# jcyk/gtos

Hardware: AMD Instinct MI355X
Metric: graphs/sec training step (100-node AMR, batch 64) (higher is better)
Workload: dtype bf16

## Files before the change

### gtos_amd/csrc/gemm.hip

```cpp
#include "common.h"
#include <stdlib.h>

__attribute__((visibility("hidden"))) const void* gtos_zero_block() {
    static void* z = nullptr;
    if (!z) {
        if (hipMalloc(&z, 256) != hipSuccess) return nullptr;
        if (hipMemset(z, 0, 256) != hipSuccess) return nullptr;
    }
    return z;
}

namespace {

constexpr int BM = 128, BN = 128;
constexpr int ROWB = 128;

template <typename T> struct GemmCfg;
template <> struct GemmCfg<bf16_t> { static constexpr int BK = 64, VEC = 8; };
template <> struct GemmCfg<float>  { static constexpr int BK = 32, VEC = 4; };

template <int NTH> struct TCfg {
    static constexpr int NT = NTH, WAVES_N = NTH / 128, WTN = BN / WAVES_N, NTW = WTN / 16;
    static constexpr int ITERS = 1024 / NTH;
};

inline const void* zero_block() { return gtos_zero_block(); }

struct GemmArgs {
    const void* A; const void* B; void* C; const float* bias;
    int M, N, K; int64_t lda, ldb, ldc;
    int vecA, vecB, vecC;
    int relu, accumulate, splitk;
    float p_drop; uint64_t seed;
    const void* zeros;
    float* ws;
};

__device__ __forceinline__ int swz(int row) { return ((row >> 1) & 7) ^ ((row >> 4) & 3); }
__device__ __forceinline__ int lds_off(int r, int c) { return r * ROWB + ((c ^ swz(r)) << 4); }

template <typename T, bool KC, bool FAST, int NTH>
__device__ __forceinline__ void load_tile(const T* __restrict__ base, const U128* __restrict__ zeros, int64_t ld, int rows_total,
                                          int row0, int k0, int kend, U128 (&regs)[TCfg<NTH>::ITERS]) {
    constexpr int VEC = GemmCfg<T>::VEC, NT = NTH, ITERS = TCfg<NTH>::ITERS;
#pragma unroll
    for (int it = 0; it < ITERS; ++it) {
        int r, k;
        if (KC) { const int v = it * NT + threadIdx.x; r = row0 + (v >> 3); k = k0 + (v & 7) * VEC; }
        else {
            const int rc = threadIdx.x % (BM / VEC), kq = threadIdx.x / (BM / VEC);
            r = row0 + rc * VEC; k = k0 + kq * ITERS + it;
        }
        if constexpr (FAST) {
            const bool ok = KC ? (r < rows_total && k + VEC <= kend) : (k < kend && r + VEC <= rows_total);
            const int64_t off = KC ? ((int64_t)r * ld + k) : ((int64_t)k * ld + r);
            const U128* p = ok ? reinterpret_cast<const U128*>(base + off) : zeros;
            regs[it] = *p;
        } else {
            U128 val = {0u, 0u, 0u, 0u};
#pragma unroll
            for (int i = 0; i < VEC; ++i) {
                const bool ok = KC ? (r < rows_total && k + i < kend) : (k < kend && r + i < rows_total);
                uint32_t bits = 0u;
                if (ok) {
                    const T x = KC ? base[(int64_t)r * ld + k + i] : base[(int64_t)k * ld + r + i];
                    if constexpr (sizeof(T) == 2) bits = (uint32_t)x; else bits = __float_as_uint(x);
                }
                if constexpr (sizeof(T) == 2) val[i >> 1] |= bits << (16 * (i & 1)); else val[i] = bits;
            }
            regs[it] = val;
        }
    }
}

template <typename T, int NTH>
__device__ __forceinline__ void glds_tile(const T* __restrict__ base, const U128* __restrict__ zeros, int64_t ld, int rows_total,
                                          int row0, int k0, int kend, char* lds_tile) {
    constexpr int VEC = GemmCfg<T>::VEC, NT = NTH, ITERS = TCfg<NTH>::ITERS;
    const int wave = __builtin_amdgcn_readfirstlane(threadIdx.x >> 6), lane = threadIdx.x & 63;
#pragma unroll
    for (int it = 0; it < ITERS; ++it) {
        const int blk = it * (NT / 64) + wave;
        const int rl = blk * 8 + (lane >> 3);
        const int c = (lane & 7) ^ swz(rl);
        const int r = row0 + rl, k = k0 + c * VEC;
        const bool ok = r < rows_total && k + VEC <= kend;
        const void* src = ok ? static_cast<const void*>(base + (int64_t)r * ld + k) : static_cast<const void*>(zeros);
        __builtin_amdgcn_global_load_lds((const __attribute__((address_space(1))) void*)src,
                                         (__attribute__((address_space(3))) void*)(lds_tile + blk * 1024), 16, 0, 0);
    }
}

typedef __attribute__((ext_vector_type(4))) short s16x4_t;

template <typename T, int NTH>
__device__ __forceinline__ void glds_tile_km(const T* __restrict__ base, const U128* __restrict__ zeros, int64_t ld, int rows_total,
                                             int row0, int k0, int kend, char* lds_tile) {
    static_assert(sizeof(T) == 2, "transpose-read path is bf16 only");
    constexpr int NT = NTH, ITERS = TCfg<NTH>::ITERS;
    const int wave = __builtin_amdgcn_readfirstlane(threadIdx.x >> 6), lane = threadIdx.x & 63;
#pragma unroll
    for (int it = 0; it < ITERS; ++it) {
        const int blk = it * (NT / 64) + wave;
        const int kr = lane >> 4, pp = lane & 15;
        const int lp = ((((pp >> 1) ^ kr) & 7) << 1) | (pp & 1);
        const int k = k0 + blk * 4 + kr, r = row0 + lp * 8;
        const bool ok = k < kend && r + 8 <= rows_total;
        const void* src = ok ? static_cast<const void*>(base + (int64_t)k * ld + r) : static_cast<const void*>(zeros);
        __builtin_amdgcn_global_load_lds((const __attribute__((address_space(1))) void*)src,
                                         (__attribute__((address_space(3))) void*)(lds_tile + blk * 1024), 16, 0, 0);
    }
}

__device__ __forceinline__ bf16x8_t tr_fragment(const char* tile, int c0, int ks, int fr, int fq) {
    const int kq = fr >> 2;
    const int col = (((c0 >> 4) ^ kq) << 5) + (fr & 3) * 8;
    const char* p0 = tile + (ks * 32 + fq * 8 + kq) * 256 + col;
    const s16x4_t lo = __builtin_amdgcn_ds_read_tr16_b64_v4i16((__attribute__((address_space(3))) s16x4_t*)(p0));
    const s16x4_t hi = __builtin_amdgcn_ds_read_tr16_b64_v4i16((__attribute__((address_space(3))) s16x4_t*)(p0 + 4 * 256));
    const s16x8_t v = {lo[0], lo[1], lo[2], lo[3], hi[0], hi[1], hi[2], hi[3]};
    return __builtin_bit_cast(bf16x8_t, v);
}

template <typename T, bool KC, int NTH>
__device__ __forceinline__ void store_tile(char* __restrict__ lds, const U128 (&regs)[TCfg<NTH>::ITERS]) {
    constexpr int VEC = GemmCfg<T>::VEC, NT = NTH, ITERS = TCfg<NTH>::ITERS;
    if (KC) {
#pragma unroll
        for (int it = 0; it < ITERS; ++it) {
            const int v = it * NT + threadIdx.x;
            *reinterpret_cast<U128*>(lds + lds_off(v >> 3, v & 7)) = regs[it];
        }
    } else {
        const int rc = threadIdx.x % (BM / VEC), kq = threadIdx.x / (BM / VEC);
        const int kk = kq * ITERS;
        if constexpr (sizeof(T) == 2) {
#pragma unroll
            for (int i = 0; i < 8; ++i) {
                const int w = i >> 1;
                char* dst = lds + lds_off(rc * 8 + i, kk >> 3) + (kk & 7) * 2;
                uint32_t lo, hi = 0u;
                if (i & 1) lo = (regs[0][w] >> 16) | (regs[1][w] & 0xffff0000u);
                else       lo = (regs[0][w] & 0xffffu) | (regs[1][w] << 16);
                if constexpr (ITERS == 4) {
                    if (i & 1) hi = (regs[2][w] >> 16) | (regs[3][w] & 0xffff0000u);
                    else       hi = (regs[2][w] & 0xffffu) | (regs[3][w] << 16);
                    *reinterpret_cast<uint2*>(dst) = make_uint2(lo, hi);
                } else {
                    *reinterpret_cast<uint32_t*>(dst) = lo;
                }
            }
        } else {
#pragma unroll
            for (int i = 0; i < 4; ++i) {
                char* dst = lds + lds_off(rc * 4 + i, kk >> 2) + (kk & 3) * 4;
                if constexpr (ITERS == 4) {
                    const U128 o = {regs[0][i], regs[1][i], regs[2][i], regs[3][i]};
                    *reinterpret_cast<U128*>(dst) = o;
                } else {
                    *reinterpret_cast<uint2*>(dst) = make_uint2(regs[0][i], regs[1][i]);
                }
            }
        }
    }
}

template <typename T, typename TO, bool TA, bool TB, bool FAST, int NTH, int STAGES>
__global__ __launch_bounds__(NTH, 4) void gemm_kernel(GemmArgs a) {
    if (a.p_drop > 0.f) a.seed = live_seed(a.seed);
    constexpr int BK = GemmCfg<T>::BK;
    constexpr int NT = NTH, WAVES_N = TCfg<NTH>::WAVES_N, WTN = TCfg<NTH>::WTN, NTW = TCfg<NTH>::NTW, ITERS = TCfg<NTH>::ITERS;
    constexpr int STAGE = (BM + BN) * ROWB;
    constexpr bool BF = sizeof(T) == 2;
    constexpr bool GA = FAST && (!TA || BF), GB = FAST && (TB || BF);
    constexpr bool TRA = GA && TA, TRB = GB && !TB;
    __shared__ __attribute__((aligned(16))) char lds[STAGES * STAGE];

    const int lane = threadIdx.x & 63, wave = threadIdx.x >> 6;
    const int wm = (wave / WAVES_N) * 64, wn = (wave % WAVES_N) * WTN;
    const int nN = (a.N + BN - 1) / BN;
    int m0, n0, bz;
    const int xcd = blockIdx.x & 7, sq = blockIdx.x >> 3;
    if (a.splitk > 1) {
        const int nM = (a.M + BM - 1) / BM, tiles = nM * nN;
        bz = (sq / tiles) * 8 + xcd;
        const int t = sq % tiles;
        m0 = (t / nN) * BM; n0 = (t % nN) * BN;
        if (bz >= a.splitk) return;
    } else {
        bz = 0;
        m0 = ((sq / nN) * 8 + xcd) * BM; n0 = (sq % nN) * BN;
        if (m0 >= a.M) return;
    }
    const int ktiles = (a.K + BK - 1) / BK;
    const int tps = (ktiles + a.splitk - 1) / a.splitk;
    const int kbeg = bz * tps * BK;
    const int kend = min(a.K, kbeg + tps * BK);
    if (kbeg >= kend && a.splitk > 1) return;

    const T* A = static_cast<const T*>(a.A);
    const T* B = static_cast<const T*>(a.B);
    const U128* Z = static_cast<const U128*>(a.zeros);

    f32x4_t acc[4][NTW];
#pragma unroll
    for (int i = 0; i < 4; ++i)
#pragma unroll
        for (int j = 0; j < NTW; ++j) acc[i][j] = f32x4_t{0.f, 0.f, 0.f, 0.f};

    const int fr = lane & 15, fq = lane >> 4;
    auto dma_a = [&](int k0x, char* dst) {
        if constexpr (TRA) glds_tile_km<T, NTH>(A, Z, a.lda, a.M, m0, k0x, kend, dst);
        else glds_tile<T, NTH>(A, Z, a.lda, a.M, m0, k0x, kend, dst);
    };
    auto dma_b = [&](int k0x, char* dst) {
        if constexpr (TRB) glds_tile_km<T, NTH>(B, Z, a.ldb, a.N, n0, k0x, kend, dst);
        else glds_tile<T, NTH>(B, Z, a.ldb, a.N, n0, k0x, kend, dst);
    };
    auto mma_stage = [&](const char* As, const char* Bs) {
        if constexpr (sizeof(T) == 2) {
#pragma unroll
            for (int ks = 0; ks < 2; ++ks) {
                bf16x8_t fa[4], fb[NTW];
#pragma unroll
                for (int t = 0; t < 4; ++t) {
                    if constexpr (TRA) fa[t] = tr_fragment(As, wm + t * 16, ks, fr, fq);
                    else fa[t] = *reinterpret_cast<const bf16x8_t*>(As + lds_off(wm + t * 16 + fr, ks * 4 + fq));
                }
#pragma unroll
                for (int t = 0; t < NTW; ++t) {
                    if constexpr (TRB) fb[t] = tr_fragment(Bs, wn + t * 16, ks, fr, fq);
                    else fb[t] = *reinterpret_cast<const bf16x8_t*>(Bs + lds_off(wn + t * 16 + fr, ks * 4 + fq));
                }
#pragma unroll
                for (int mt = 0; mt < 4; ++mt)
#pragma unroll
                    for (int nt = 0; nt < NTW; ++nt)
                        acc[mt][nt] = __builtin_amdgcn_mfma_f32_16x16x32_bf16(fb[nt], fa[mt], acc[mt][nt], 0, 0, 0);
            }
        } else {
#pragma unroll
            for (int ks = 0; ks < 8; ++ks) {
                float fa[4], fb[NTW];
#pragma unroll
                for (int t = 0; t < 4; ++t) fa[t] = *reinterpret_cast<const float*>(As + lds_off(wm + t * 16 + fr, ks) + fq * 4);
#pragma unroll
                for (int t = 0; t < NTW; ++t) fb[t] = *reinterpret_cast<const float*>(Bs + lds_off(wn + t * 16 + fr, ks) + fq * 4);
#pragma unroll
                for (int mt = 0; mt < 4; ++mt)
#pragma unroll
                    for (int nt = 0; nt < NTW; ++nt)
                        acc[mt][nt] = __builtin_amdgcn_mfma_f32_16x16x4f32(fb[nt], fa[mt], acc[mt][nt], 0, 0, 0);
            }
        }
    };

    if constexpr (STAGES == 1) {
        static_assert(!(STAGES == 1) || (GA && GB), "single-stage variant needs both operands by DMA");
        if constexpr (!TRA && !TRB) {
            const char* Ab = reinterpret_cast<const char*>(A + (int64_t)m0 * a.lda);
            const char* Bb = reinterpret_cast<const char*>(B + (int64_t)n0 * a.ldb);
            const int amax = a.M - 1 - m0, bmax = a.N - 1 - n0;
            const uint32_t lda2 = (uint32_t)a.lda * (uint32_t)sizeof(T), ldb2 = (uint32_t)a.ldb * (uint32_t)sizeof(T);
            const int wv = __builtin_amdgcn_readfirstlane(threadIdx.x >> 6);
            uint32_t offA[ITERS], offB[ITERS];
            int cc[ITERS];
#pragma unroll
            for (int it = 0; it < ITERS; ++it) {
                const int rl = (it * (NT / 64) + wv) * 8 + (lane >> 3);
                cc[it] = (lane & 7) ^ swz(rl);
                offA[it] = (uint32_t)min(rl, amax) * lda2 + (uint32_t)(cc[it] << 4);
                offB[it] = (uint32_t)min(rl, bmax) * ldb2 + (uint32_t)(cc[it] << 4);
            }
            constexpr int VEC = GemmCfg<T>::VEC;
            for (int k0 = kbeg; k0 < kend; k0 += BK) {
                const char* ak = Ab + (int64_t)k0 * (int)sizeof(T);
                const char* bk = Bb + (int64_t)k0 * (int)sizeof(T);
                if (k0 + BK <= kend) {
#pragma unroll
                    for (int it = 0; it < ITERS; ++it) {
                        const int blk = it * (NT / 64) + wv;
                        __builtin_amdgcn_global_load_lds((const __attribute__((address_space(1))) void*)(ak + offA[it]),
                                                         (__attribute__((address_space(3))) void*)(lds + blk * 1024), 16, 0, 0);
                        __builtin_amdgcn_global_load_lds((const __attribute__((address_space(1))) void*)(bk + offB[it]),
                                                         (__attribute__((address_space(3))) void*)(lds + BM * ROWB + blk * 1024), 16, 0, 0);
                    }
                } else {
#pragma unroll
                    for (int it = 0; it < ITERS; ++it) {
                        const int blk = it * (NT / 64) + wv;
                        const bool ok = k0 + cc[it] * VEC + VEC <= kend;
                        const void* sa = ok ? static_cast<const void*>(ak + offA[it]) : static_cast<const void*>(Z);
                        const void* sb = ok ? static_cast<const void*>(bk + offB[it]) : static_cast<const void*>(Z);
                        __builtin_amdgcn_global_load_lds((const __attribute__((address_space(1))) void*)sa,
                                                         (__attribute__((address_space(3))) void*)(lds + blk * 1024), 16, 0, 0);
                        __builtin_amdgcn_global_load_lds((const __attribute__((address_space(1))) void*)sb,
                                                         (__attribute__((address_space(3))) void*)(lds + BM * ROWB + blk * 1024), 16, 0, 0);
                    }
                }
                __syncthreads();
                mma_stage(lds, lds + BM * ROWB);
                __syncthreads();
            }
        } else {
        for (int k0 = kbeg; k0 < kend; k0 += BK) {
            dma_a(k0, lds);
            dma_b(k0, lds + BM * ROWB);
            __syncthreads();
            mma_stage(lds, lds + BM * ROWB);
            __syncthreads();
        }
        }
    } else {
    U128 ra0[ITERS], rb0[ITERS], ra1[ITERS], rb1[ITERS];
    if constexpr (GA) dma_a(kbeg, lds);
    else { load_tile<T, !TA, FAST, NTH>(A, Z, a.lda, a.M, m0, kbeg, kend, ra0); store_tile<T, !TA, NTH>(lds, ra0);
           load_tile<T, !TA, FAST, NTH>(A, Z, a.lda, a.M, m0, kbeg + BK, kend, ra0); }
    if constexpr (GB) dma_b(kbeg, lds + BM * ROWB);
    else { load_tile<T, TB, FAST, NTH>(B, Z, a.ldb, a.N, n0, kbeg, kend, rb0); store_tile<T, TB, NTH>(lds + BM * ROWB, rb0);
           load_tile<T, TB, FAST, NTH>(B, Z, a.ldb, a.N, n0, kbeg + BK, kend, rb0); }
    __syncthreads();

    int cur = 0;
    for (int k0 = kbeg; k0 < kend; k0 += 2 * BK) {
        {
            const char* As = lds + cur * STAGE;
            char* An = lds + (cur ^ 1) * STAGE;
            if constexpr (GA) dma_a(k0 + BK, An);
            else load_tile<T, !TA, FAST, NTH>(A, Z, a.lda, a.M, m0, k0 + 2 * BK, kend, ra1);
            if constexpr (GB) dma_b(k0 + BK, An + BM * ROWB);
            else load_tile<T, TB, FAST, NTH>(B, Z, a.ldb, a.N, n0, k0 + 2 * BK, kend, rb1);
            __builtin_amdgcn_sched_barrier(0);
            mma_stage(As, As + BM * ROWB);
            __builtin_amdgcn_sched_barrier(0);
            if constexpr (!GA) store_tile<T, !TA, NTH>(An, ra0);
            if constexpr (!GB) store_tile<T, TB, NTH>(An + BM * ROWB, rb0);
            __syncthreads();
            cur ^= 1;
        }
        if (k0 + BK >= kend) break;
        {
            const char* As = lds + cur * STAGE;
            char* An = lds + (cur ^ 1) * STAGE;
            if constexpr (GA) dma_a(k0 + 2 * BK, An);
            else load_tile<T, !TA, FAST, NTH>(A, Z, a.lda, a.M, m0, k0 + 3 * BK, kend, ra0);
            if constexpr (GB) dma_b(k0 + 2 * BK, An + BM * ROWB);
            else load_tile<T, TB, FAST, NTH>(B, Z, a.ldb, a.N, n0, k0 + 3 * BK, kend, rb0);
            __builtin_amdgcn_sched_barrier(0);
            mma_stage(As, As + BM * ROWB);
            __builtin_amdgcn_sched_barrier(0);
            if constexpr (!GA) store_tile<T, !TA, NTH>(An, ra1);
            if constexpr (!GB) store_tile<T, TB, NTH>(An + BM * ROWB, rb1);
            __syncthreads();
            cur ^= 1;
        }
    }

    }

    TO* C = static_cast<TO*>(a.C);
    const float keep_scale = a.p_drop > 0.f ? 1.f / (1.f - a.p_drop) : 1.f;

    if constexpr (sizeof(TO) == 2) {
        if (a.vecC && a.splitk == 1) {
            constexpr int CP = WTN * 2 + 16;
            constexpr int LPR = WTN / 8, RPP = 64 / LPR;
            char* cs = lds + wave * 32 * CP;
            if (!a.bias && !a.relu && !(a.p_drop > 0.f) && !a.accumulate && m0 + BM <= a.M && n0 + BN <= a.N) {
                const int rrow = lane / LPR, rcol = (lane % LPR) * 8;
                char* wr = cs + fr * CP + fq * 8;
                const char* rd = cs + rrow * CP + rcol * 2;
                bf16_t* cp0 = reinterpret_cast<bf16_t*>(C) + (int64_t)(m0 + wm + rrow) * a.ldc + n0 + wn + rcol;
#pragma unroll
                for (int half = 0; half < 2; ++half) {
#pragma unroll
                    for (int mh = 0; mh < 2; ++mh)
#pragma unroll
                        for (int nt = 0; nt < NTW; ++nt) {
                            const f32x4_t v = acc[half * 2 + mh][nt];
                            *reinterpret_cast<uint2*>(wr + mh * 16 * CP + nt * 32) = make_uint2(pack_bf(v[0], v[1]), pack_bf(v[2], v[3]));
                        }
                    __builtin_amdgcn_fence(__ATOMIC_RELEASE, "wavefront");
                    __builtin_amdgcn_s_waitcnt(0xc07f);
#pragma unroll
                    for (int pass = 0; pass < 32 / RPP; ++pass) {
                        const uint4 val = *reinterpret_cast<const uint4*>(rd + pass * RPP * CP);
                        *reinterpret_cast<uint4*>(cp0 + (int64_t)(half * 32 + pass * RPP) * a.ldc) = val;
                    }
                    __builtin_amdgcn_s_waitcnt(0xc07f);
                }
                return;
            }
#pragma unroll
            for (int half = 0; half < 2; ++half) {
                if (half) __syncthreads();
#pragma unroll
                for (int mh = 0; mh < 2; ++mh)
#pragma unroll
                    for (int nt = 0; nt < NTW; ++nt) {
                        const int mt = half * 2 + mh;
                        const int m = m0 + wm + mt * 16 + fr, n = n0 + wn + nt * 16 + fq * 4;
                        float v[4] = {acc[mt][nt][0], acc[mt][nt][1], acc[mt][nt][2], acc[mt][nt][3]};
#pragma unroll
                        for (int i = 0; i < 4; ++i) {
                            if (a.bias && n + i < a.N) v[i] += a.bias[n + i];
                            if (a.relu) v[i] = fmaxf(v[i], 0.f);
                            if (a.p_drop > 0.f)
                                v[i] = drop_keep(a.seed, (uint64_t)m * (uint64_t)a.N + (uint64_t)(n + i), a.p_drop) ? v[i] * keep_scale : 0.f;
                        }
                        *reinterpret_cast<uint2*>(cs + (mh * 16 + fr) * CP + (nt * 16 + fq * 4) * 2) =
                            make_uint2(pack_bf(v[0], v[1]), pack_bf(v[2], v[3]));
                    }
                __syncthreads();
#pragma unroll
                for (int pass = 0; pass < 32 / RPP; ++pass) {
                    const int row = pass * RPP + lane / LPR, col = (lane % LPR) * 8;
                    const int m = m0 + wm + half * 32 + row, n = n0 + wn + col;
                    if (m >= a.M || n >= a.N) continue;
                    uint4 val = *reinterpret_cast<const uint4*>(cs + row * CP + col * 2);
                    bf16_t* cp = reinterpret_cast<bf16_t*>(C) + (int64_t)m * a.ldc + n;
                    if (n + 8 <= a.N) {
                        if (a.accumulate) {
                            const uint4 old = *reinterpret_cast<const uint4*>(cp);
                            val = make_uint4(pack_bf(lo_bf(val.x) + lo_bf(old.x), hi_bf(val.x) + hi_bf(old.x)),
                                             pack_bf(lo_bf(val.y) + lo_bf(old.y), hi_bf(val.y) + hi_bf(old.y)),
                                             pack_bf(lo_bf(val.z) + lo_bf(old.z), hi_bf(val.z) + hi_bf(old.z)),
                                             pack_bf(lo_bf(val.w) + lo_bf(old.w), hi_bf(val.w) + hi_bf(old.w)));
                        }
                        *reinterpret_cast<uint4*>(cp) = val;
                    } else {
                        const bf16_t* e = reinterpret_cast<const bf16_t*>(cs + row * CP + col * 2);
                        for (int i = 0; i < 8 && n + i < a.N; ++i) {
                            float o = bf2f(e[i]);
                            if (a.accumulate) o += bf2f(cp[i]);
                            cp[i] = f2bf(o);
                        }
                    }
                }
            }
            return;
        }
    }

#pragma unroll
    for (int mt = 0; mt < 4; ++mt) {
        const int m = m0 + wm + mt * 16 + fr;
        if (m >= a.M) continue;
#pragma unroll
        for (int nt = 0; nt < NTW; ++nt) {
            const int n = n0 + wn + nt * 16 + fq * 4;
            if (n >= a.N) continue;
            float v[4] = {acc[mt][nt][0], acc[mt][nt][1], acc[mt][nt][2], acc[mt][nt][3]};
            TO* cp = C + (int64_t)m * a.ldc + n;
            if (a.splitk > 1) {
                if constexpr (sizeof(TO) == 4) {
                    if (a.ws) {
                        *reinterpret_cast<float4*>(a.ws + ((int64_t)bz * a.M + m) * a.N + n) = make_float4(v[0], v[1], v[2], v[3]);
                    } else {
#pragma unroll
                        for (int i = 0; i < 4; ++i) if (n + i < a.N) atomicAdd(reinterpret_cast<float*>(cp) + i, v[i]);
                    }
                }
                continue;
            }
#pragma unroll
            for (int i = 0; i < 4; ++i) {
                if (a.bias && n + i < a.N) v[i] += a.bias[n + i];
                if (a.relu) v[i] = fmaxf(v[i], 0.f);
                if (a.p_drop > 0.f)
                    v[i] = drop_keep(a.seed, (uint64_t)m * (uint64_t)a.N + (uint64_t)(n + i), a.p_drop) ? v[i] * keep_scale : 0.f;
            }
            if (sizeof(TO) == 4 && a.vecC && n + 3 < a.N) {
                float4 o = make_float4(v[0], v[1], v[2], v[3]);
                if (a.accumulate) { const float4 c = *reinterpret_cast<const float4*>(cp); o.x += c.x; o.y += c.y; o.z += c.z; o.w += c.w; }
                *reinterpret_cast<float4*>(cp) = o;
            } else {
#pragma unroll
                for (int i = 0; i < 4; ++i) if (n + i < a.N) {
                    float o = v[i];
                    if (a.accumulate) o += to_f<TO>(cp[i]);
                    cp[i] = from_f<TO>(o);
                }
            }
        }
    }
}

__global__ void splitk_reduce_kernel(const float* __restrict__ ws, int splits, int M, int N, float* __restrict__ C, int64_t ldc) {
    const int64_t n4 = N / 4, total = (int64_t)M * n4, plane = (int64_t)M * N;
    for (int64_t t = (int64_t)blockIdx.x * blockDim.x + threadIdx.x; t < total; t += (int64_t)gridDim.x * blockDim.x) {
        const int m = (int)(t / n4), n = (int)(t % n4) * 4;
        const float* p = ws + (int64_t)m * N + n;
        float4 acc = *reinterpret_cast<const float4*>(p);
        for (int s = 1; s < splits; ++s) {
            const float4 v = *reinterpret_cast<const float4*>(p + s * plane);
            acc.x += v.x; acc.y += v.y; acc.z += v.z; acc.w += v.w;
        }
        float* cp = C + (int64_t)m * ldc + n;
        cp[0] += acc.x; cp[1] += acc.y; cp[2] += acc.z; cp[3] += acc.w;
    }
}


constexpr int BM2 = 256, BN2 = 256, STAGE2 = (BM2 + BN2) * ROWB;
const bool g_use256 = !(getenv("GTOS_GEMM256") && getenv("GTOS_GEMM256")[0] == '0');

__global__ __launch_bounds__(512, 2) void gemm256_nt_kernel(GemmArgs a) {
    if (a.p_drop > 0.f) a.seed = live_seed(a.seed);
    extern __shared__ __attribute__((aligned(16))) char lds2[];
    const int lane = threadIdx.x & 63, wave = __builtin_amdgcn_readfirstlane(threadIdx.x >> 6);
    const int fr = lane & 15, fq = lane >> 4;
    const int wm = (wave >> 2) * 128, wn = (wave & 3) * 64;
// ... 386 lines not shown
        GTOS_DMA1(ok0 ? pb : Z, (stage) + A3 + wave * 1024);                                                                  \
        GTOS_DMA1(ok1 ? pb + b16 : Z, (stage) + A3 + (8 + wave) * 1024);                                                      \
        kcur += 32; pa += 2 * a16; pb += 2 * b16;                                                                             \
    }
#define GTOS_TRF(tile, c0)                                                                                                    \
    ([&]() -> bf16x8_t {                                                                                                      \
        const char* p0 = (tile) + fbase + ((((c0) >> 4) ^ kq) << 5);                                                          \
        const s16x4_t lo = __builtin_amdgcn_ds_read_tr16_b64_v4i16((__attribute__((address_space(3))) s16x4_t*)(p0));         \
        const s16x4_t hi = __builtin_amdgcn_ds_read_tr16_b64_v4i16((__attribute__((address_space(3))) s16x4_t*)(p0 + 4 * 512)); \
        const s16x8_t v = {lo[0], lo[1], lo[2], lo[3], hi[0], hi[1], hi[2], hi[3]};                                           \
        return __builtin_bit_cast(bf16x8_t, v);                                                                               \
    }())
#define GTOS_STEP(slot_s, slot_d, s_)                                                                                         \
    {                                                                                                                         \
        GTOS_DMA4(slot_d);                                                                                                  \
        _Pragma("unroll") for (int t = 0; t < 4; ++t) fb[t] = GTOS_TRF((slot_s) + A3, wn + t * 16);                           \
        _Pragma("unroll") for (int t = 0; t < 8; ++t) fa[t] = GTOS_TRF((slot_s), wm + t * 16);                                \
        __builtin_amdgcn_s_waitcnt(0x0078);                 \
        __builtin_amdgcn_s_barrier();                                                                                         \
        __builtin_amdgcn_sched_barrier(0);                                                                                    \
        _Pragma("unroll") for (int mt = 0; mt < 8; ++mt)                                                                      \
            _Pragma("unroll") for (int nt = 0; nt < 4; ++nt)                                                                  \
                acc[mt][nt] = __builtin_amdgcn_mfma_f32_16x16x32_bf16(fb[nt], fa[mt], acc[mt][nt], 0, 0, 0);                  \
        __builtin_amdgcn_sched_barrier(0);                                                                                    \
        __builtin_amdgcn_s_barrier();                                                                                         \
    }

    GTOS_DMA4(st0);
    GTOS_DMA4(st1);
    GTOS_DMA4(st2);
    GTOS_VMCNT(8);
    __builtin_amdgcn_s_barrier();
    if (wave >= 4) __builtin_amdgcn_s_barrier();
    int s = 0;
    for (; s + 4 <= nk; s += 4) {
        GTOS_STEP(st0, st3, s);
        GTOS_STEP(st1, st0, s + 1);
        GTOS_STEP(st2, st1, s + 2);
        GTOS_STEP(st3, st2, s + 3);
    }
    if (s < nk) {
        GTOS_STEP(st0, st3, s);
        if (s + 1 < nk) {
            GTOS_STEP(st1, st0, s + 1);
            if (s + 2 < nk) GTOS_STEP(st2, st1, s + 2);
        }
    }
    if (wave < 4) __builtin_amdgcn_s_barrier();
#undef GTOS_STEP
#undef GTOS_TRF
#undef GTOS_DMA4
#undef GTOS_DMA1

#pragma unroll
    for (int mt = 0; mt < 8; ++mt) {
        const int m = m0 + wm + mt * 16 + fr;
        if (m >= a.M) continue;
#pragma unroll
        for (int nt = 0; nt < 4; ++nt) {
            const int n = n0 + wn + nt * 16 + fq * 4;
            if (n >= Nv) continue;
            float4* dst = reinterpret_cast<float4*>(wst + (int64_t)(m - m0) * wld + (n - n0));
            if constexpr (MODE == 2) {
                const float4 o = *dst;
                *dst = make_float4(o.x + acc[mt][nt][0], o.y + acc[mt][nt][1], o.z + acc[mt][nt][2], o.w + acc[mt][nt][3]);
            } else {
                *dst = make_float4(acc[mt][nt][0], acc[mt][nt][1], acc[mt][nt][2], acc[mt][nt][3]);
            }
        }
    }
}

struct ColJob { const bf16_t* A; float* out; int lda, M, K, blk_end, gx; };
struct ColBatch { int njobs, nblocks, rpb; ColJob job[TN_MAX_JOBS]; };
__global__ __launch_bounds__(256) void colsum_batch_kernel(ColBatch g) {
    __shared__ float red[4][64][8];
    int t_ = blockIdx.x, j = 0;
    if (t_ >= g.nblocks) return;
    while (j + 1 < g.njobs && t_ >= g.job[j].blk_end) ++j;
    const ColJob& jb = g.job[j];
    const int tl = t_ - (j ? g.job[j - 1].blk_end : 0);
    const int bx = tl % jb.gx, by = tl / jb.gx;
    const int lane = threadIdx.x & 63, w = threadIdx.x >> 6;
    const int c = (bx * 64 + lane) * 8;
    const int r0 = by * g.rpb, r1 = min(jb.K, r0 + g.rpb);
    float acc[8] = {0, 0, 0, 0, 0, 0, 0, 0};
    if (c < jb.M) {
        for (int r = r0 + w; r < r1; r += 4) {
            float v[8];
            Vec8<bf16_t>::load(jb.A + (int64_t)r * jb.lda + c, v);
#pragma unroll
            for (int e = 0; e < 8; ++e) acc[e] += v[e];
        }
    }
#pragma unroll
    for (int e = 0; e < 8; ++e) red[w][lane][e] = acc[e];
    __syncthreads();
    if (w == 0 && c < jb.M) {
#pragma unroll
        for (int e = 0; e < 8; ++e) atomicAdd(jb.out + c + e, red[0][lane][e] + red[1][lane][e] + red[2][lane][e] + red[3][lane][e]);
    }
}

struct GruDwOut { float* dwih; int64_t ld_ih; float* dwhh; int64_t ld_hh; int hs, in_dim; };
__global__ void gru_dw_reduce_kernel(const float* __restrict__ ws, int splits, TnGroup g, GruDwOut o) {
    const int t_ = blockIdx.x >> 6, q = (blockIdx.x & 63) * 256 + threadIdx.x;
    const int e = g.tmn[t_], src = (e >> 8) & 255;
    const int r = q >> 6, c = (q & 63) * 4;
    const int i = (e & 255) * BM2 + r, j = ((e >> 16) & 255) * BN2 + c;
    if (i >= 4 * o.hs) return;
    const int gate = i / o.hs, ch = i - gate * o.hs;
    float* dst;
    if (src == 0) {
        if (gate == 3 || j >= o.in_dim) return;
        dst = o.dwih + (int64_t)(gate * o.hs + ch) * o.ld_ih + j;
    } else {
        if (gate == 2 || j >= o.hs) return;
        dst = o.dwhh + (int64_t)((gate == 3 ? 2 : gate) * o.hs + ch) * o.ld_hh + j;
    }
    const float* p = ws + (int64_t)t_ * (BM2 * BN2) + r * BN2 + c;
    const int64_t plane = (int64_t)g.tiles * (BM2 * BN2);
    float4 acc = *reinterpret_cast<const float4*>(p);
    for (int s = 1; s < splits; ++s) {
        const float4 v = *reinterpret_cast<const float4*>(p + s * plane);
        acc.x += v.x; acc.y += v.y; acc.z += v.z; acc.w += v.w;
    }
    dst[0] += acc.x; dst[1] += acc.y; dst[2] += acc.z; dst[3] += acc.w;
}

int launch256p_tn(const GemmArgs& a, hipStream_t s) {
    const long long tiles = ((long long)(a.M + BM2 - 1) / BM2) * ((a.N + BN2 - 1) / BN2);
    const long long nblk = tiles * 8 * ((a.splitk + 7) / 8);
    if (nblk > 0x7fffffffLL) return -6;
    hipLaunchKernelGGL((gemm256p_tn_kernel<0, TnGroup>), dim3((unsigned)nblk), dim3(512), 0, s, a, TnGroup{});
    GTOS_CHECK_LAUNCH();
    return 0;
}

int launch256(const GemmArgs& a, hipStream_t s) {
    static bool configured = false;
    if (!configured) {
        if (hipFuncSetAttribute(reinterpret_cast<const void*>(gemm256_nt_kernel), hipFuncAttributeMaxDynamicSharedMemorySize,
                                2 * STAGE2) != hipSuccess) return -7;
        configured = true;
    }
    const long long nMt = (a.M + BM2 - 1) / BM2, nNt = (a.N + BN2 - 1) / BN2;
    const long long nblk = ((nMt + 7) / 8) * 8 * nNt;
    if (nblk > 0x7fffffffLL) return -6;
    hipLaunchKernelGGL(gemm256_nt_kernel, dim3((unsigned)nblk), dim3(512), 2 * STAGE2, s, a);
    GTOS_CHECK_LAUNCH();
    return 0;
}

template <typename T, typename TO>
int launch(const GemmArgs& a, int transA, int transB, hipStream_t s) {
    const long long nMt = (a.M + BM - 1) / BM, nNt = (a.N + BN - 1) / BN;
    const long long nblk = a.splitk > 1 ? nMt * nNt * 8 * ((a.splitk + 7) / 8) : ((nMt + 7) / 8) * 8 * nNt;
    if (nblk > 0x7fffffffLL) return -6;
    dim3 grid((unsigned)nblk);
    const bool fast = a.vecA && a.vecB;
    constexpr bool BF = sizeof(T) == 2;
    if (!transA && transB) {
        if (fast) hipLaunchKernelGGL((gemm_kernel<T, TO, false, true, true, 256, 1>), grid, dim3(256), 0, s, a);
        else      hipLaunchKernelGGL((gemm_kernel<T, TO, false, true, false, 512, 2>), grid, dim3(512), 0, s, a);
    } else if (!transA && !transB) {
        if (fast && BF) hipLaunchKernelGGL((gemm_kernel<T, TO, false, false, true, 256, BF ? 1 : 2>), grid, dim3(256), 0, s, a);
        else if (fast)  hipLaunchKernelGGL((gemm_kernel<T, TO, false, false, true, 512, 2>), grid, dim3(512), 0, s, a);
        else            hipLaunchKernelGGL((gemm_kernel<T, TO, false, false, false, 512, 2>), grid, dim3(512), 0, s, a);
    } else if (transA && !transB) {
        if (fast && BF) hipLaunchKernelGGL((gemm_kernel<T, TO, true, false, true, 256, BF ? 1 : 2>), grid, dim3(256), 0, s, a);
        else if (fast)  hipLaunchKernelGGL((gemm_kernel<T, TO, true, false, true, 512, 2>), grid, dim3(512), 0, s, a);
        else            hipLaunchKernelGGL((gemm_kernel<T, TO, true, false, false, 512, 2>), grid, dim3(512), 0, s, a);
    } else return -2;
    GTOS_CHECK_LAUNCH();
    return 0;
}

}

extern "C" int gtos_gemm(int in_dtype, int out_dtype, int transA, int transB, int M, int N, int K,
                         const void* A, int64_t lda, const void* B, int64_t ldb, void* C, int64_t ldc,
                         const float* bias, int relu, float p_drop, uint64_t seed, int accumulate,
                         int splitk, void* workspace, int64_t workspace_bytes, void* stream) {
    if (M <= 0 || N <= 0) return 0;
    if (K <= 0) return -3;
    const int es = in_dtype == GTOS_BF16 ? 2 : 4, vec = 16 / es;
    const int eo = out_dtype == GTOS_BF16 ? 2 : 4;
    GemmArgs a;
    a.A = A; a.B = B; a.C = C; a.bias = bias; a.M = M; a.N = N; a.K = K; a.lda = lda; a.ldb = ldb; a.ldc = ldc;
    a.vecA = ((uintptr_t)A % 16 == 0) && (lda % vec == 0) && ((transA ? M : K) % vec == 0);
    a.vecB = ((uintptr_t)B % 16 == 0) && (ldb % vec == 0) && ((transB ? K : N) % vec == 0);
    a.vecC = ((uintptr_t)C % 16 == 0) && (ldc % (16 / eo) == 0);
    a.relu = relu; a.accumulate = accumulate; a.p_drop = p_drop; a.seed = seed;
    a.zeros = zero_block();
    if (!a.zeros) return -5;
    if (splitk < 1) splitk = 1;
    const int BKc = in_dtype == GTOS_BF16 ? GemmCfg<bf16_t>::BK : GemmCfg<float>::BK;
    const int ktiles = (K + BKc - 1) / BKc;
    if (splitk > ktiles) splitk = ktiles;
    if (splitk > 1) { const int tps = (ktiles + splitk - 1) / splitk; splitk = (ktiles + tps - 1) / tps; }
    a.splitk = splitk;
    if (splitk > 1 && (out_dtype != GTOS_F32 || bias || relu || p_drop > 0.f || !accumulate)) return -4;
    hipStream_t s = static_cast<hipStream_t>(stream);
    a.ws = nullptr;
    if (splitk > 1 && workspace && N % 4 == 0 && (uintptr_t)workspace % 16 == 0 && (uintptr_t)C % 4 == 0 &&
        (int64_t)splitk * M * N * 4 <= workspace_bytes) {
        a.ws = static_cast<float*>(workspace);
        const int kps = ((ktiles + splitk - 1) / splitk) * BKc;
        const bool tn256 = g_use_pipe_tn && in_dtype == GTOS_BF16 && transA && !transB && a.vecA && a.vecB && M >= 256 && N >= 256 &&
                           M % 8 == 0 && N % 8 == 0 && kps >= 256;
        int rc = tn256 ? launch256p_tn(a, s)
                       : (in_dtype == GTOS_BF16 ? launch<bf16_t, float>(a, transA, transB, s) : launch<float, float>(a, transA, transB, s));
        if (rc) return rc;
        const int64_t total = (int64_t)M * (N / 4);
        const int nb = (int)((total + 255) / 256 < 2048 ? (total + 255) / 256 : 2048);
        hipLaunchKernelGGL(splitk_reduce_kernel, dim3(nb), dim3(256), 0, s, a.ws, splitk, M, N, static_cast<float*>(C), ldc);
        GTOS_CHECK_LAUNCH();
        return 0;
    }
    if (in_dtype == GTOS_BF16 && out_dtype == GTOS_BF16) {
        const long long t256 = ((long long)(M + BM2 - 1) / BM2) * ((N + BN2 - 1) / BN2);
        if (g_use_pipe && !transA && transB && a.vecA && a.vecB && a.vecC && splitk == 1 && N >= 256 && K % 32 == 0 &&
            lda < (1 << 22) && ldb < (1 << 22) &&
            (t256 >= 512 && K >= g_min_kpipe))
            return launch256p(a, s);
        if (g_use256 && !transA && transB && a.vecA && a.vecB && a.vecC && splitk == 1 && t256 >= 1024 && N >= 256 && K >= g_min_k256)
            return launch256(a, s);
        return launch<bf16_t, bf16_t>(a, transA, transB, s);
    }
    if (in_dtype == GTOS_BF16 && out_dtype == GTOS_F32)  return launch<bf16_t, float>(a, transA, transB, s);
    if (in_dtype == GTOS_F32 && out_dtype == GTOS_F32)   return launch<float, float>(a, transA, transB, s);
    return -1;
}


extern "C" int gtos_gru_weight_grads(int rows, int hs, int in_dim, int in_valid, const void* d4, const void* x, int64_t ldx, const void* hprev, int64_t ldh,
                                     float* dwih, int64_t ld_dwih, float* dwhh, int64_t ld_dwhh, void* workspace, int64_t workspace_bytes,
                                     void* stream) {
    if (rows <= 0) return 0;
    if (hs <= 0 || hs % 64 || in_dim < 8 || in_dim % 8 || ldx < in_dim || ldx % 8 || ldh < hs || ldh % 8 || in_valid < 1 || in_valid > in_dim ||
        in_valid % 4) return -22;
    if (!d4 || !x || !hprev || !dwih || !dwhh || !workspace) return -23;
    if ((uintptr_t)d4 % 16 || (uintptr_t)x % 16 || (uintptr_t)hprev % 16 || (uintptr_t)dwih % 4 || (uintptr_t)dwhh % 4 || (uintptr_t)workspace % 16 ||
        ld_dwih < in_valid || ld_dwhh < hs) return -25;
    GemmArgs a{};
    a.A = d4; a.lda = 4 * (int64_t)hs; a.M = 4 * hs; a.B = x; a.ldb = ldx; a.N = in_dim; a.K = rows; a.vecA = a.vecB = 1;
    a.accumulate = 1; a.zeros = zero_block();
    if (!a.zeros) return -5;
    TnGroup g{};
    g.B1 = static_cast<const bf16_t*>(hprev); g.ldb1 = ldh; g.N1 = hs;
    int nt = 0;
    for (int mb = 0; mb * BM2 < 4 * hs; ++mb) {
        const int lo = mb * BM2, hi = (lo + BM2 < 4 * hs ? lo + BM2 : 4 * hs) - 1;
        const int g_lo = lo / hs, g_hi = hi / hs;
        const bool needs_x = g_lo <= 2, needs_h = !(g_lo == 2 && g_hi == 2);
        for (int src = 0; src < 2; ++src) {
            if (!(src ? needs_h : needs_x)) continue;
            const int ncols = src ? hs : in_dim;
            for (int nb = 0; nb * BN2 < ncols; ++nb) {
                if (nt >= 64) return -28;
                g.tmn[nt++] = mb | (src << 8) | (nb << 16);
            }
        }
    }
    g.tiles = nt;
    const int ktiles = (rows + 63) / 64;
    const long long tile_bytes = (long long)BM2 * BN2 * 4;
    long long sk = 8LL * (32 / nt > 0 ? 32 / nt : 1);
    if (sk > ktiles / 4) sk = ktiles / 4;
    if (sk * nt * tile_bytes > workspace_bytes) sk = workspace_bytes / (nt * tile_bytes);
    if (sk < 1) { if (nt * tile_bytes > workspace_bytes) return -4; sk = 1; }
    const int tps = (int)((ktiles + sk - 1) / sk);
    a.splitk = (ktiles + tps - 1) / tps;
    a.ws = static_cast<float*>(workspace);
    hipStream_t s = static_cast<hipStream_t>(stream);
    const long long nblk = (long long)nt * 8 * ((a.splitk + 7) / 8);
    hipLaunchKernelGGL((gemm256p_tn_kernel<1, TnGroup>), dim3((unsigned)nblk), dim3(512), 0, s, a, g);
    GTOS_CHECK_LAUNCH();
    GruDwOut o{dwih, ld_dwih, dwhh, ld_dwhh, hs, in_valid};
    hipLaunchKernelGGL(gru_dw_reduce_kernel, dim3((unsigned)(nt * 64)), dim3(256), 0, s, a.ws, a.splitk, g, o);
    GTOS_CHECK_LAUNCH();
    return 0;
}

extern "C" int gtos_gemm_tn_batch(int n, const void* const* A, const int64_t* lda, const int* M, const void* const* B, const int64_t* ldb,
                                  const int* N, const int* K, float* const* C, const int64_t* ldc, float* const* bias, void* stream) {
    if (n <= 0) return 0;
    if (!A || !lda || !M || !B || !ldb || !N || !K || !C || !ldc) return -23;
    hipStream_t s = static_cast<hipStream_t>(stream);
    const void* zeros = zero_block();
    if (!zeros) return -5;
    for (int j = 0; j < n; ++j) {
        if (M[j] < 8 || M[j] % 8 || N[j] < 8 || N[j] % 8 || K[j] < 1 || lda[j] < M[j] || lda[j] % 8 || ldb[j] < N[j] || ldb[j] % 8 || ldc[j] < N[j] ||
            ldc[j] % 4 || lda[j] >= (1LL << 31) || ldb[j] >= (1LL << 31) || ldc[j] >= (1LL << 31)) return -22;
        if (!A[j] || !B[j] || !C[j] || (uintptr_t)A[j] % 16 || (uintptr_t)B[j] % 16 || (uintptr_t)C[j] % 16) return -25;
        if (bias && bias[j] && (uintptr_t)bias[j] % 4) return -25;
    }
    for (int j0 = 0, nj = 0; j0 < n; j0 += nj) {
        nj = 0;
        while (nj < TN_MAX_JOBS && j0 + nj < n) {
            const int q = j0 + nj;
            const uintptr_t lo = (uintptr_t)C[q], hi = lo + (uintptr_t)(((int64_t)(M[q] - 1) * ldc[q] + N[q]) * 4);
            bool meets = false;
            for (int p = j0; p < q && !meets; ++p) {
                const uintptr_t plo = (uintptr_t)C[p], phi = plo + (uintptr_t)(((int64_t)(M[p] - 1) * ldc[p] + N[p]) * 4);
                meets = lo < phi && plo < hi;
            }
            if (meets) break;
            ++nj;
        }
        TnBatch tb{};
        ColBatch cb{};
        int tiles = 0, blocks = 0, ncol = 0;
        cb.rpb = 512;
        for (int j = 0; j < nj; ++j) {
            const int q = j0 + j;
            TnJob& t = tb.job[j];
            t.A = static_cast<const bf16_t*>(A[q]); t.B = static_cast<const bf16_t*>(B[q]); t.C = C[q];
            t.lda = (int)lda[q]; t.ldb = (int)ldb[q]; t.ldc = (int)ldc[q]; t.M = M[q]; t.N = N[q]; t.K = K[q];
            t.nN = (N[q] + BN2 - 1) / BN2;
            tiles += ((M[q] + BM2 - 1) / BM2) * t.nN;
            t.tile_end = tiles;
            if (bias && bias[q]) {
                ColJob& c = cb.job[ncol++];
                c.A = t.A; c.out = bias[q]; c.lda = t.lda; c.M = t.M; c.K = t.K;
                c.gx = (t.M + 511) / 512;
                blocks += c.gx * ((t.K + cb.rpb - 1) / cb.rpb);
                c.blk_end = blocks;
            }
        }
        tb.njobs = nj; tb.ntiles = tiles;
        GemmArgs a{};
        a.splitk = 1; a.zeros = zeros; a.vecA = a.vecB = 1; a.accumulate = 1;
        hipLaunchKernelGGL((gemm256p_tn_kernel<2, TnBatch>), dim3((unsigned)tiles), dim3(512), 0, s, a, tb);
        GTOS_CHECK_LAUNCH();
        if (ncol) {
            cb.njobs = ncol; cb.nblocks = blocks;
            hipLaunchKernelGGL(colsum_batch_kernel, dim3((unsigned)blocks), dim3(256), 0, s, cb);
            GTOS_CHECK_LAUNCH();
        }
    }
    return 0;
}

GTOS_SEED_EPOCH_SETTER(gemm)
```

Baseline: 850.3.

## Add multi-stage ring-buffered NT GEMM kernel for small-grid bf16 GEMMs

Adds a new 128x128 NT GEMM kernel that keeps a 3- or 4-slot LDS ring filled by direct global-to-LDS loads. Each step waits with a partial vmcnt so several K tiles stay in flight while MFMA runs on the oldest slot. It is routed for bf16 NT GEMMs whose grid is small (by default 128 workgroups or fewer), where the existing kernels cannot hide memory latency through occupancy. The epilogue is moved into a shared device function so both kernels use it. The change adds env-var lookups on every GEMM call and a launch counter. It also statically allocates four LDS stages even when only three are used, which may limit occupancy.

```diff
diff --git a/gtos_amd/csrc/gemm.hip b/gtos_amd/csrc/gemm.hip
--- a/gtos_amd/csrc/gemm.hip
+++ b/gtos_amd/csrc/gemm.hip
@@ -164,6 +164,9 @@
         }
     }
 }
+
+template <typename TO, int NTH>
+__device__ __forceinline__ void gemm_epilogue(const GemmArgs& a, const f32x4_t (&acc)[4][TCfg<NTH>::NTW], char* lds, int m0, int n0, int bz);
 
 template <typename T, typename TO, bool TA, bool TB, bool FAST, int NTH, int STAGES>
 __global__ __launch_bounds__(NTH, 4) void gemm_kernel(GemmArgs a) {
@@ -358,6 +361,15 @@
 
     }
 
+    gemm_epilogue<TO, NTH>(a, acc, lds, m0, n0, bz);
+}
+
+template <typename TO, int NTH>
+__device__ __forceinline__ void gemm_epilogue(const GemmArgs& a, const f32x4_t (&acc)[4][TCfg<NTH>::NTW], char* lds, int m0, int n0, int bz) {
+    constexpr int WAVES_N = TCfg<NTH>::WAVES_N, WTN = TCfg<NTH>::WTN, NTW = TCfg<NTH>::NTW;
+    const int lane = threadIdx.x & 63, wave = threadIdx.x >> 6;
+    const int wm = (wave / WAVES_N) * 64, wn = (wave % WAVES_N) * WTN;
+    const int fr = lane & 15, fq = lane >> 4;
     TO* C = static_cast<TO*>(a.C);
     const float keep_scale = a.p_drop > 0.f ? 1.f / (1.f - a.p_drop) : 1.f;
 
@@ -1050,6 +1062,141 @@
     return 0;
 }
 
+constexpr int RSTAGE = (BM + BN) * ROWB;
+
+template <typename TO, int NS>
+__global__ __launch_bounds__(256) void gemm_ring_nt_kernel(GemmArgs a) {
+    static_assert(NS == 3 || NS == 4, "ring of three or four stages");
+    if (a.p_drop > 0.f) a.seed = live_seed(a.seed);
+    __shared__ __attribute__((aligned(16))) char r0[RSTAGE];
+    __shared__ __attribute__((aligned(16))) char r1[RSTAGE];
+    __shared__ __attribute__((aligned(16))) char r2[RSTAGE];
+    __shared__ __attribute__((aligned(16))) char r3[RSTAGE];
+    const int lane = threadIdx.x & 63, wv = __builtin_amdgcn_readfirstlane(threadIdx.x >> 6);
+    const int fr = lane & 15, fq = lane >> 4;
+    const int wm = (wv >> 1) * 64, wn = (wv & 1) * 64;
+    const int nN = (a.N + BN - 1) / BN;
+    const int xcd = blockIdx.x & 7, sq = blockIdx.x >> 3;
+    const int m0 = ((sq / nN) * 8 + xcd) * BM, n0 = (sq % nN) * BN;
+    if (m0 >= a.M) return;
+    const char* Ab = reinterpret_cast<const char*>(static_cast<const bf16_t*>(a.A) + (int64_t)m0 * a.lda);
+    const char* Bb = reinterpret_cast<const char*>(static_cast<const bf16_t*>(a.B) + (int64_t)n0 * a.ldb);
+    const char* Z = static_cast<const char*>(a.zeros);
+    const int amax = a.M - 1 - m0, bmax = a.N - 1 - n0;
+    const uint32_t lda2 = (uint32_t)a.lda * 2u, ldb2 = (uint32_t)a.ldb * 2u;
+    const int nk = (a.K + 63) / 64;
+    const bool tail = (a.K & 63) != 0;
+    uint32_t offA[4], offB[4];
+    bool tz[4];
+#pragma unroll
+    for (int it = 0; it < 4; ++it) {
+        const int rl = (it * 4 + wv) * 8 + (lane >> 3);
+        const int c = (lane & 7) ^ swz(rl);
+        tz[it] = (nk - 1) * 64 + c * 8 + 8 > a.K;
+        offA[it] = (uint32_t)min(rl, amax) * lda2 + (uint32_t)(c << 4);
+        offB[it] = (uint32_t)min(rl, bmax) * ldb2 + (uint32_t)(c << 4);
+    }
+    f32x4_t acc[4][4];
+#pragma unroll
+    for (int i = 0; i < 4; ++i)
+#pragma unroll
+        for (int j = 0; j < 4; ++j) acc[i][j] = f32x4_t{0.f, 0.f, 0.f, 0.f};
+
+#define GTOS_RDMA(src, dst)                                                                                                   \
+    __builtin_amdgcn_global_load_lds((const __attribute__((address_space(1))) void*)(src),                                    \
+                                     (__attribute__((address_space(3))) void*)(dst), 16, 0, 0)
+#define GTOS_RISSUE(slot, kt_)                                                                                                \
+    {                                                                                                                         \
+        const int kc_ = min((kt_), nk - 1);                                                                                   \
+        const char* ak_ = Ab + kc_ * 128;                                                                                     \
+        const char* bk_ = Bb + kc_ * 128;                                                                                     \
+        const bool zs_ = tail && (kt_) >= nk - 1;           \
+        _Pragma("unroll") for (int it = 0; it < 4; ++it) {                                                                    \
+            GTOS_RDMA((zs_ && tz[it]) ? Z : ak_ + offA[it], (slot) + (it * 4 + wv) * 1024);                                   \
+            GTOS_RDMA((zs_ && tz[it]) ? Z : bk_ + offB[it], (slot) + BM * ROWB + (it * 4 + wv) * 1024);                       \
+        }                                                                                                                     \
+    }
+#define GTOS_RSTEP(slot_s, slot_d, kt_)                                                                                       \
+    {                                                                                                                         \
+        GTOS_VMCNT((NS - 2) * 8);                                                               \
+        __builtin_amdgcn_s_waitcnt(0xc07f);                   \
+        __builtin_amdgcn_s_barrier();                                       \
+        __builtin_amdgcn_sched_barrier(0);                                                                                    \
+        GTOS_RISSUE(slot_d, (kt_) + NS - 1);                                                                                  \
+        __builtin_amdgcn_sched_barrier(0);                                                                                    \
+        _Pragma("unroll") for (int ks = 0; ks < 2; ++ks) {                                                                    \
+            bf16x8_t fa[4], fb[4];                                                                                            \
+            _Pragma("unroll") for (int t = 0; t < 4; ++t)                                                                     \
+                fa[t] = *reinterpret_cast<const bf16x8_t*>((slot_s) + lds_off(wm + t * 16 + fr, ks * 4 + fq));                \
+            _Pragma("unroll") for (int t = 0; t < 4; ++t)                                                                     \
+                fb[t] = *reinterpret_cast<const bf16x8_t*>((slot_s) + BM * ROWB + lds_off(wn + t * 16 + fr, ks * 4 + fq));    \
+            _Pragma("unroll") for (int mt = 0; mt < 4; ++mt)                                                                  \
+                _Pragma("unroll") for (int nt = 0; nt < 4; ++nt)                                                              \
+                    acc[mt][nt] = __builtin_amdgcn_mfma_f32_16x16x32_bf16(fb[nt], fa[mt], acc[mt][nt], 0, 0, 0);              \
+        }                                                                                                                     \
+        __builtin_amdgcn_sched_barrier(0);                                                                                    \
+    }
+
+    int kt = 0;
+    if constexpr (NS == 3) {
+        GTOS_RISSUE(r0, 0);
+        GTOS_RISSUE(r1, 1);
+        for (; kt + 3 <= nk; kt += 3) {
+            GTOS_RSTEP(r0, r2, kt);
+            GTOS_RSTEP(r1, r0, kt + 1);
+            GTOS_RSTEP(r2, r1, kt + 2);
+        }
+        if (kt < nk) {
+            GTOS_RSTEP(r0, r2, kt);
+            if (kt + 1 < nk) GTOS_RSTEP(r1, r0, kt + 1);
+        }
+    } else {
+        GTOS_RISSUE(r0, 0);
+        GTOS_RISSUE(r1, 1);
+        GTOS_RISSUE(r2, 2);
+        for (; kt + 4 <= nk; kt += 4) {
+            GTOS_RSTEP(r0, r3, kt);
+            GTOS_RSTEP(r1, r0, kt + 1);
+            GTOS_RSTEP(r2, r1, kt + 2);
+            GTOS_RSTEP(r3, r2, kt + 3);
+        }
+        if (kt < nk) {
+            GTOS_RSTEP(r0, r3, kt);
+            if (kt + 1 < nk) {
+                GTOS_RSTEP(r1, r0, kt + 1);
+                if (kt + 2 < nk) GTOS_RSTEP(r2, r1, kt + 2);
+            }
+        }
+    }
+    GTOS_VMCNT(0);
+    __builtin_amdgcn_s_waitcnt(0xc07f);
+    __syncthreads();
+#undef GTOS_RSTEP
+#undef GTOS_RISSUE
+#undef GTOS_RDMA
+    gemm_epilogue<TO, 256>(a, acc, r0, m0, n0, 0);
+}
+
+constexpr int g_ring_ns = 3;
+constexpr int g_ring_max_wgs = 128;
+long long g_ring_launches = 0;
+
+inline int env_int(const char* name, int dflt) {
+    const char* v = getenv(name);
+    return v && *v ? atoi(v) : dflt;
+}
+
+template <typename TO>
+int launch_ring(const GemmArgs& a, int ns, hipStream_t s) {
+    const long long nMt = (a.M + BM - 1) / BM, nNt = (a.N + BN - 1) / BN;
+    const unsigned nblk = (unsigned)(((nMt + 7) / 8) * 8 * nNt);
+    if (ns == 3) hipLaunchKernelGGL((gemm_ring_nt_kernel<TO, 3>), dim3(nblk), dim3(256), 0, s, a);
+    else         hipLaunchKernelGGL((gemm_ring_nt_kernel<TO, 4>), dim3(nblk), dim3(256), 0, s, a);
+    GTOS_CHECK_LAUNCH();
+    ++g_ring_launches;
+    return 0;
+}
+
 template <typename T, typename TO>
 int launch(const GemmArgs& a, int transA, int transB, hipStream_t s) {
     const long long nMt = (a.M + BM - 1) / BM, nNt = (a.N + BN - 1) / BN;
@@ -1075,6 +1222,8 @@
 }
 
 }
+
+extern "C" long long gtos_gemm_ring_launches() { return g_ring_launches; }
 
 extern "C" int gtos_gemm(int in_dtype, int out_dtype, int transA, int transB, int M, int N, int K,
                          const void* A, int64_t lda, const void* B, int64_t ldb, void* C, int64_t ldc,
@@ -1116,6 +1265,13 @@
         GTOS_CHECK_LAUNCH();
         return 0;
     }
+    if (in_dtype == GTOS_BF16 && !transA && transB && a.vecA && a.vecB && a.vecC && splitk == 1 && lda < (1 << 22) && ldb < (1 << 22)) {
+        const long long wgs = (((long long)(M + BM - 1) / BM + 7) / 8) * 8 * ((N + BN - 1) / BN);
+        if (wgs <= env_int("GTOS_GEMM_RING_TILES", g_ring_max_wgs) && env_int("GTOS_GEMM_RING", 1) != 0) {
+            const int ns = env_int("GTOS_GEMM_RING_NS", g_ring_ns) == 3 ? 3 : 4;
+            return out_dtype == GTOS_BF16 ? launch_ring<bf16_t>(a, ns, s) : launch_ring<float>(a, ns, s);
+        }
+    }
     if (in_dtype == GTOS_BF16 && out_dtype == GTOS_BF16) {
         const long long t256 = ((long long)(M + BM2 - 1) / BM2) * ((N + BN2 - 1) / BN2);
         if (g_use_pipe && !transA && transB && a.vecA && a.vecB && a.vecC && splitk == 1 && N >= 256 && K % 32 == 0 &&
```

Result: no change. 854.9, median of 6 (+0.5%).
